# podmortem/operator

Hardware: AMD Instinct MI355X
Metric: pod-failure analyses/sec (whole node) + p50 explanation latency, 8B TP=1 (higher is better)
Workload: dtype bf16

## Files before the change

### csrc/bindings.cpp

```cpp
#include <torch/extension.h>
#include <c10/hip/HIPStream.h>
#include <ATen/hip/impl/HIPGuardImplMasqueradingAsCUDA.h>
#include <ATen/hip/impl/HIPStreamMasqueradingAsCUDA.h>

#include "kernels/kernels.h"
#include "kernels/scan.h"

namespace {

using oamd::bf16_t;

hipStream_t cur_stream() { return c10::hip::getCurrentHIPStreamMasqueradingAsCUDA().stream(); }

#define CHECK_DEV(t) TORCH_CHECK((t).is_cuda(), #t " must be a GPU tensor")
#define CHECK_CONTIG(t) TORCH_CHECK((t).is_contiguous(), #t " must be contiguous")
#define CHECK_DT(t, dt) TORCH_CHECK((t).scalar_type() == (dt), #t " has wrong dtype ", (t).scalar_type())
#define CHECK_BF16(t) CHECK_DT(t, at::kBFloat16)
#define ROWMAJOR_VEC(t) \
  TORCH_CHECK((t).dim() == 2 && (t).stride(1) == 1 && (t).stride(0) % 8 == 0, #t " must be [rows, cols] row-major with 16-B aligned rows")
#define RC(call)                                                           \
  do {                                                                     \
    int rc__ = (call);                                                     \
    TORCH_CHECK(rc__ == 0, "kernel launch failed: " #call " rc=", rc__);   \
  } while (0)
// ... 212 lines not shown

void gemm_tile(const at::Tensor& x, const at::Tensor& w, const c10::optional<at::Tensor>& y_opt,
               const c10::optional<at::Tensor>& bias, bool silu_gu, int64_t variant, int64_t splits,
               const c10::optional<at::Tensor>& partial) {
  CHECK_DEV(x); CHECK_BF16(x); CHECK_BF16(w); CHECK_CONTIG(x); CHECK_CONTIG(w);
  TORCH_CHECK(x.dim() == 2 && w.dim() == 2, "x [M,K], w [N,K]");
  const int64_t M = x.size(0), K = x.size(1), N = w.size(0);
  TORCH_CHECK(w.size(1) == K, "gemm_tile: w [N, K] must match x [M, K]");
  TORCH_CHECK(M >= 1 && K >= 64 && K % 64 == 0 && N % 16 == 0, "gemm_tile: K % 64 == 0, N % 16 == 0");
  TORCH_CHECK(splits >= 1 && splits <= 64 && K % (64 * splits) == 0, "gemm_tile: K % (64 * splits) == 0");
  bf16_t* yp = nullptr;
  int64_t ldy = silu_gu ? N / 2 : N;
  if (y_opt.has_value()) {
    const at::Tensor& y = *y_opt;
    CHECK_BF16(y);
    TORCH_CHECK(y.dim() == 2 && y.size(0) == M && y.size(1) == (silu_gu ? N / 2 : N) && y.stride(1) == 1 &&
                    y.stride(0) % 4 == 0,
                "gemm_tile: y [M, N] (N/2 with silu_gu), unit column stride, 8-B aligned rows");
    TORCH_CHECK(reinterpret_cast<uintptr_t>(y.data_ptr()) % 8 == 0, "gemm_tile: y must be 8-B aligned");
    TORCH_CHECK(splits == 1 || silu_gu || y.stride(0) == N, "gemm_tile: split-K reduce needs a contiguous y");
    yp = ptr<bf16_t>(y);
    ldy = y.stride(0);
  } else {
    TORCH_CHECK(splits > 1 && !silu_gu, "y may be omitted only for split-K slabs summed by the consumer");
  }
  TORCH_CHECK(!silu_gu || (N % 128 == 0 && !bias.has_value()), "gemm_tile: SwiGLU needs N % 128, no bias");
  TORCH_CHECK(splits == 1 || !bias.has_value(), "gemm_tile: no bias with split-K");
  if (bias.has_value()) {
    CHECK_BF16(*bias); CHECK_CONTIG(*bias);
    TORCH_CHECK(bias->numel() == N, "gemm_tile: bias [N]");
  }
  float* pp = nullptr;
  if (splits > 1) {
    TORCH_CHECK(partial.has_value(), "gemm_tile: split-K needs a partial buffer");
    CHECK_DT(*partial, at::kFloat); CHECK_CONTIG(*partial);
    TORCH_CHECK(partial->numel() >= splits * M * N, "gemm_tile: partial buffer too small");
    pp = partial->data_ptr<float>();
  }
  TORCH_CHECK(M * K < (1LL << 40) && N * K < (1LL << 40) && M < (1LL << 31) && N < (1LL << 31), "gemm too large");
  const c10::hip::HIPGuardMasqueradingAsCUDA g(x.device());
  RC(oamd::gemm_tile(ptr<bf16_t>(x), ptr<bf16_t>(w), yp, optr<bf16_t>(bias), (int)M, (int)N, (int)K, (int)ldy,
                     silu_gu, (int)variant, (int)splits, pp, cur_stream()));
}

void gemm_pp(const at::Tensor& x, const at::Tensor& w, const c10::optional<at::Tensor>& y_opt,
             const c10::optional<at::Tensor>& p, int64_t splits, int64_t bm, bool silu_gu, bool nt, bool one_seg,
             const c10::optional<at::Tensor>& sk_ws, const c10::optional<at::Tensor>& sk_flags) {
  CHECK_DEV(x); CHECK_BF16(x); CHECK_BF16(w); CHECK_CONTIG(x); CHECK_CONTIG(w);
  TORCH_CHECK(x.dim() == 2 && w.dim() == 2 && w.size(1) == x.size(1), "x [M,K], w [N,K]");
  const int64_t M = x.size(0), K = x.size(1), N = w.size(0);
  TORCH_CHECK(M >= 1 && N % 128 == 0, "gemm_pp: N % 128 == 0");
  TORCH_CHECK(bm == 128 || bm == 256, "gemm_pp: bm in {128, 256}");
  TORCH_CHECK(splits >= 1 && splits <= 32 && K % (64 * splits) == 0, "gemm_pp: K % (64 * splits) == 0");
  TORCH_CHECK(!silu_gu || splits == 1, "gemm_pp: fused SwiGLU needs splits == 1");
  bf16_t* yp = nullptr;
  if (y_opt.has_value()) {
    CHECK_BF16(*y_opt); CHECK_CONTIG(*y_opt);
    TORCH_CHECK(y_opt->dim() == 2 && y_opt->size(0) == M && y_opt->size(1) == (silu_gu ? N / 2 : N), "gemm_pp: y");
    yp = ptr<bf16_t>(*y_opt);
  } else {
    TORCH_CHECK(splits > 1 && !silu_gu, "y may be omitted only for split-K slabs summed by the consumer");
  }
  float* pp = nullptr;
  if (splits > 1) {
    TORCH_CHECK(p.has_value(), "split-K needs a partial buffer");
    CHECK_DT(*p, at::kFloat); CHECK_CONTIG(*p);
    TORCH_CHECK(p->numel() >= splits * M * N, "partial buffer too small");
    pp = p->data_ptr<float>();
  }
  TORCH_CHECK(M * K < (1LL << 40) && N * K < (1LL << 40), "gemm too large");
  const c10::hip::HIPGuardMasqueradingAsCUDA g(x.device());
  float* wsp = nullptr;
  int* flp = nullptr;
  if (sk_ws.has_value() || sk_flags.has_value()) {
    TORCH_CHECK(sk_ws.has_value() && sk_flags.has_value(), "gemm_pp: stream-K needs sk_ws and sk_flags");
    CHECK_DEV(*sk_ws); CHECK_DEV(*sk_flags); CHECK_CONTIG(*sk_ws); CHECK_CONTIG(*sk_flags);
    CHECK_DT(*sk_ws, at::kFloat); CHECK_DT(*sk_flags, at::kInt);
    TORCH_CHECK(sk_ws->numel() >= (N / 128) * 32768 && sk_flags->numel() >= N / 128, "gemm_pp: stream-K workspace too small");
    wsp = sk_ws->data_ptr<float>();
    flp = sk_flags->data_ptr<int>();
  }
  RC(oamd::gemm_pp(ptr<bf16_t>(x), ptr<bf16_t>(w), yp, pp, (int)M, (int)N, (int)K, (int)splits, (int)bm, silu_gu, nt,
                   cur_stream(), one_seg, wsp, flp));
}

void gemm_skinny(const at::Tensor& x, const at::Tensor& w, const c10::optional<at::Tensor>& y_opt,
                 const c10::optional<at::Tensor>& p, int64_t splits, bool silu_gu) {
  CHECK_DEV(x); CHECK_BF16(x); CHECK_BF16(w); CHECK_CONTIG(x); CHECK_CONTIG(w);
  TORCH_CHECK(x.dim() == 2 && w.dim() == 2 && w.size(1) == x.size(1), "x [M,K], w [N,K]");
  const int64_t M = x.size(0), K = x.size(1), N = w.size(0);
  TORCH_CHECK(M >= 1 && M <= 32, "gemm_skinny: M must be 1..32");
  TORCH_CHECK(N % (silu_gu ? 128 : 16) == 0, "gemm_skinny: N % 16 (128 for the fused SwiGLU)");
  TORCH_CHECK(splits >= 1 && splits <= 8 && K % (128 * splits) == 0, "gemm_skinny: K % (128 * splits)");
  TORCH_CHECK(!silu_gu || splits == 1, "fused SwiGLU needs splits = 1");
  bf16_t* yp = nullptr;
  if (y_opt.has_value()) {
    CHECK_BF16(*y_opt); CHECK_CONTIG(*y_opt);
    TORCH_CHECK(y_opt->dim() == 2 && y_opt->size(0) == M && y_opt->size(1) == (silu_gu ? N / 2 : N), "gemm shapes");
    yp = ptr<bf16_t>(*y_opt);
  } else {
    TORCH_CHECK(splits > 1 && !silu_gu, "y may be omitted only for split-K slabs summed by the consumer");
  }
  float* pp = nullptr;
  if (splits > 1) {
    TORCH_CHECK(p.has_value(), "split-K needs a partial buffer");
    CHECK_DT(*p, at::kFloat); CHECK_CONTIG(*p);
    TORCH_CHECK(p->numel() >= splits * M * N, "partial buffer too small");
    TORCH_CHECK((M * N) % 4 == 0 || yp == nullptr, "split-K reduce needs M * N % 4 == 0");
    pp = p->data_ptr<float>();
  }
  TORCH_CHECK(N * K < (1LL << 40) && M * K < (1LL << 31), "gemm too large");
  const c10::hip::HIPGuardMasqueradingAsCUDA g(x.device());
  RC(oamd::gemm_skinny(ptr<bf16_t>(x), ptr<bf16_t>(w), yp, pp, (int)M, (int)N, (int)K, (int)splits, silu_gu,
                       cur_stream()));
}

void quantize_fp8(const at::Tensor& x, at::Tensor& q, at::Tensor& sx) {
  CHECK_DEV(x); CHECK_BF16(x); CHECK_CONTIG(q); CHECK_CONTIG(sx); CHECK_DT(sx, at::kFloat);
  TORCH_CHECK(x.dim() == 2 && x.stride(1) == 1, "x must be [M, K] row-major");
  TORCH_CHECK(q.scalar_type() == at::kByte || q.scalar_type() == at::kFloat8_e4m3fn, "q must be uint8 / e4m3fn");
  const int64_t M = x.size(0), K = x.size(1);
  TORCH_CHECK(q.numel() == M * K && sx.numel() == M && K % 8 == 0, "quantize_fp8 shapes");
  const c10::hip::HIPGuardMasqueradingAsCUDA g(x.device());
  RC(oamd::quantize_fp8_rows(ptr<bf16_t>(x), static_cast<uint8_t*>(q.data_ptr()), ptr<float>(sx), (int)M, (int)K,
                             x.stride(0), cur_stream()));
}

void silu_quantize_fp8(const at::Tensor& gu, at::Tensor& q, at::Tensor& sx, const c10::optional<at::Tensor>& slabs,
                       int64_t splits) {
  CHECK_DEV(gu); CHECK_CONTIG(q); CHECK_CONTIG(sx); CHECK_DT(sx, at::kFloat);
  TORCH_CHECK(gu.dim() == 2 && gu.stride(1) == 1, "gu must be [M, 2I] row-major");
  TORCH_CHECK(q.scalar_type() == at::kByte || q.scalar_type() == at::kFloat8_e4m3fn, "q must be uint8 / e4m3fn");
  const int64_t M = gu.size(0), I = gu.size(1) / 2;
  TORCH_CHECK(gu.size(1) % 128 == 0 && I <= 16384, "silu_quantize_fp8: 2I % 128 == 0, I <= 16384");
  TORCH_CHECK(q.numel() == M * I && sx.numel() == M, "silu_quantize_fp8 shapes");
  const float* pp = nullptr;
  if (slabs.has_value()) {
    CHECK_DT(*slabs, at::kFloat); CHECK_CONTIG(*slabs);
    TORCH_CHECK(splits >= 1 && slabs->numel() >= splits * M * 2 * I, "slabs: fp32 [splits, M, 2I]");
    pp = slabs->data_ptr<float>();
  } else {
    CHECK_BF16(gu);
  }
  const c10::hip::HIPGuardMasqueradingAsCUDA g(gu.device());
  RC(oamd::silu_quantize_fp8(pp != nullptr ? nullptr : ptr<bf16_t>(gu), pp, (int)splits,
                             static_cast<uint8_t*>(q.data_ptr()), ptr<float>(sx), (int)M, (int)I,
                             pp != nullptr ? 2 * I : gu.stride(0), cur_stream()));
}

void gemm_fp8(const at::Tensor& x8, const at::Tensor& w8, const at::Tensor& sx, const at::Tensor& sw, at::Tensor& y,
              const c10::optional<at::Tensor>& p, int64_t splits, int64_t bn, int64_t bm, bool reduce) {
  CHECK_DEV(x8); CHECK_CONTIG(x8); CHECK_CONTIG(w8); CHECK_CONTIG(sx); CHECK_CONTIG(sw); CHECK_BF16(y);
  CHECK_CONTIG(y); CHECK_DT(sx, at::kFloat); CHECK_DT(sw, at::kFloat);
  for (auto* t : {&x8, &w8})
    TORCH_CHECK(t->scalar_type() == at::kByte || t->scalar_type() == at::kFloat8_e4m3fn, "fp8 operands");
  TORCH_CHECK(x8.dim() == 2 && w8.dim() == 2, "x8 [M,K], w8 [N,K]");
  const int64_t M = x8.size(0), K = x8.size(1), N = w8.size(0);
  TORCH_CHECK(w8.size(1) == K && y.size(0) == M && y.size(1) == N && sx.numel() == M && sw.numel() == N,
              "gemm_fp8 shapes");
  TORCH_CHECK((bn == 64 || bn == 128) && N % bn == 0, "gemm_fp8: N % bn");
  TORCH_CHECK(bm == 64 || bm == 128 || bm == 256, "gemm_fp8: bm in {64,128,256}");
  TORCH_CHECK(splits >= 1 && splits <= 16 && K % 128 == 0 && K / 128 >= splits, "gemm_fp8: K % 128, 1 <= splits <= min(16, K / 128)");
  float* pp = nullptr;
  if (splits > 1) {
    TORCH_CHECK(p.has_value() && p->scalar_type() == at::kFloat && p->numel() >= splits * M * N,
                "split-K needs an fp32 partial buffer");
// ... 150 lines not shown
                        ptr<int>(work_seq), ptr<int>(work_q0), (int)work_seq.numel(), (int)q.size(1),
                        (int)k.size(1), 128, (float)scale, (int)variant, cur_stream(), pkp, pvp, pfx));
}

void sample(const at::Tensor& logits, const at::Tensor& temperature, const at::Tensor& seeds,
            const at::Tensor& positions, at::Tensor& out, int64_t col_offset,
            const c10::optional<at::Tensor>& out_val) {
  CHECK_DEV(logits);
  TORCH_CHECK(logits.dim() == 2 && logits.stride(1) == 1, "logits must be [rows, vocab] row-major");
  TORCH_CHECK(logits.scalar_type() == at::kFloat || logits.scalar_type() == at::kBFloat16, "logits dtype");
  const int64_t rows = logits.size(0);
  CHECK_DT(temperature, at::kFloat); CHECK_DT(seeds, at::kLong); CHECK_DT(positions, at::kLong); CHECK_DT(out, at::kLong);
  TORCH_CHECK(temperature.numel() == rows && seeds.numel() == rows && positions.numel() == rows && out.numel() == rows,
              "sampler per-row tensor shape");
  if (out_val.has_value()) {
    CHECK_DT(*out_val, at::kFloat);
    TORCH_CHECK(out_val->numel() == rows, "out_val shape");
  }
  const c10::hip::HIPGuardMasqueradingAsCUDA g(logits.device());
  RC(oamd::sample_tokens(logits.data_ptr(), logits.scalar_type() == at::kBFloat16, logits.stride(0), (int)rows,
                         (int)logits.size(1), ptr<float>(temperature), ptr<int64_t>(seeds), ptr<int64_t>(positions),
                         ptr<int64_t>(out), col_offset, optr<float>(out_val), cur_stream()));
}

}

void graph_launch(int64_t exec, int64_t count, int64_t stream) {
  TORCH_CHECK(exec != 0 && count >= 0, "graph_launch: bad graph / count");
  hipError_t err = hipSuccess;
  {
    pybind11::gil_scoped_release nogil;
    for (int64_t i = 0; i < count && err == hipSuccess; ++i)
      err = hipGraphLaunch(reinterpret_cast<hipGraphExec_t>(exec), reinterpret_cast<hipStream_t>(stream));
  }
  TORCH_CHECK(err == hipSuccess, "hipGraphLaunch failed: ", hipGetErrorString(err));
}

void register_scan_bindings(pybind11::module_& m);
void register_comm_bindings(pybind11::module_& m);

PYBIND11_MODULE(_C, m) {
  m.doc() = "operator_amd gfx950 kernels";
  m.def("rmsnorm", &rmsnorm, "RMSNorm with optional fused residual add (and split-K slab sum)", pybind11::arg("x"),
        pybind11::arg("residual"), pybind11::arg("w"), pybind11::arg("y"), pybind11::arg("eps"),
        pybind11::arg("partial") = pybind11::none(), pybind11::arg("splits") = 1, pybind11::arg("tiled_out") = false);
  m.def("gemm_xr", &gemm_xr, pybind11::arg("xt"), pybind11::arg("w"), pybind11::arg("y") = pybind11::none(),
        pybind11::arg("p") = pybind11::none(), pybind11::arg("splits") = 1, pybind11::arg("epi") = 1);
  m.def("tile_rows", &tile_rows, pybind11::arg("x"), pybind11::arg("xt"));
  m.def("silu_mul", &silu_mul, pybind11::arg("gu"), pybind11::arg("out"), pybind11::arg("block") = 0);
  m.def("embedding", &embedding);
  m.def("rope_kv", &rope_kv, pybind11::arg("qkv"), pybind11::arg("pos"), pybind11::arg("cos"),
        pybind11::arg("sin"), pybind11::arg("Hq"), pybind11::arg("Hkv"), pybind11::arg("q_out"),
        pybind11::arg("k_out"), pybind11::arg("v_out"), pybind11::arg("k_cache"), pybind11::arg("v_cache"),
        pybind11::arg("slots"), pybind11::arg("partial") = pybind11::none(), pybind11::arg("splits") = 1,
        pybind11::arg("bias") = pybind11::none(), pybind11::arg("k_scale") = 1.0, pybind11::arg("v_scale") = 1.0);
  m.def("attn_decode", &attn_decode, pybind11::arg("q"), pybind11::arg("k_cache"), pybind11::arg("v_cache"),
        pybind11::arg("block_tables"), pybind11::arg("seq_lens"), pybind11::arg("out"), pybind11::arg("o_part"),
        pybind11::arg("ml_part"), pybind11::arg("num_splits"), pybind11::arg("scale"), pybind11::arg("variant") = 0,
        pybind11::arg("k_scale") = 1.0, pybind11::arg("v_scale") = 1.0, pybind11::arg("q8") = pybind11::none(),
        pybind11::arg("sx") = pybind11::none(), pybind11::arg("rope_x") = pybind11::none(),
        pybind11::arg("rope_splits") = 1, pybind11::arg("pos") = pybind11::none(), pybind11::arg("cos") = pybind11::none(),
        pybind11::arg("sin") = pybind11::none(), pybind11::arg("slots") = pybind11::none(),
        pybind11::arg("bias") = pybind11::none());
  m.def("decode_slots", &decode_slots);
  m.def("decode_advance", &decode_advance);
  m.def("quantize_fp8", &quantize_fp8);
  m.def("silu_quantize_fp8", &silu_quantize_fp8, pybind11::arg("gu"), pybind11::arg("q"), pybind11::arg("sx"),
        pybind11::arg("slabs") = pybind11::none(), pybind11::arg("splits") = 1);
  m.def("score_events", &score_events);
  m.def("gemm_fp8", &gemm_fp8, pybind11::arg("x8"), pybind11::arg("w8"), pybind11::arg("sx"), pybind11::arg("sw"),
        pybind11::arg("y"), pybind11::arg("p") = pybind11::none(), pybind11::arg("splits") = 1,
        pybind11::arg("bn") = 64, pybind11::arg("bm") = 64, pybind11::arg("reduce") = true);
  m.def("gemm_decode", &gemm_decode, pybind11::arg("x"), pybind11::arg("w"), pybind11::arg("y"),
        pybind11::arg("p") = pybind11::none(), pybind11::arg("splits") = 1, pybind11::arg("bn") = 64,
        pybind11::arg("bm") = 0, pybind11::arg("silu_gu") = false, pybind11::arg("w_tiled") = false,
        pybind11::arg("stages") = 3);
  m.def("gemm_tile", &gemm_tile, pybind11::arg("x"), pybind11::arg("w"), pybind11::arg("y"),
        pybind11::arg("bias") = pybind11::none(), pybind11::arg("silu_gu") = false, pybind11::arg("variant") = 0,
        pybind11::arg("splits") = 1, pybind11::arg("partial") = pybind11::none());
  m.def("gemm_pp", &gemm_pp, pybind11::arg("x"), pybind11::arg("w"), pybind11::arg("y"),
        pybind11::arg("p") = pybind11::none(), pybind11::arg("splits") = 1, pybind11::arg("bm") = 256,
        pybind11::arg("silu_gu") = false, pybind11::arg("nt") = true, pybind11::arg("one_seg") = false,
        pybind11::arg("sk_ws") = pybind11::none(), pybind11::arg("sk_flags") = pybind11::none());
  m.def("gemm_pp_sk_grid", &oamd::gemm_pp_sk_grid, pybind11::arg("tiles"), pybind11::arg("steps"));
  m.def("gemm_skinny", &gemm_skinny, pybind11::arg("x"), pybind11::arg("w"), pybind11::arg("y"),
        pybind11::arg("p") = pybind11::none(), pybind11::arg("splits") = 1, pybind11::arg("silu_gu") = false);
  m.def("attn_prefill", &attn_prefill, pybind11::arg("q"), pybind11::arg("k"), pybind11::arg("v"),
        pybind11::arg("o"), pybind11::arg("cu_seqlens"), pybind11::arg("work_seq"), pybind11::arg("work_q0"),
        pybind11::arg("scale"), pybind11::arg("block_q") = 64, pybind11::arg("pk") = pybind11::none(),
        pybind11::arg("pv") = pybind11::none(), pybind11::arg("seq_pfx") = pybind11::none());
  m.def("attn_prefill_block_q", &oamd::attn_prefill_block_q);
  m.def("sample", &sample, pybind11::arg("logits"), pybind11::arg("temperature"), pybind11::arg("seeds"),
        pybind11::arg("positions"), pybind11::arg("out"), pybind11::arg("col_offset") = 0,
        pybind11::arg("out_val") = pybind11::none());
  m.def("graph_launch", &graph_launch, pybind11::arg("graph_exec"), pybind11::arg("count"), pybind11::arg("stream"));
  register_scan_bindings(m);
  register_comm_bindings(m);
  m.attr("ARCH") = "gfx950";
}
```

### csrc/kernels/kernels.h

```cpp
#pragma once
#include <hip/hip_runtime.h>
#include <stdint.h>

namespace oamd {
typedef uint16_t bf16_t;

int rmsnorm(const bf16_t* x, bf16_t* residual, const bf16_t* w, bf16_t* y, int rows, int hidden,
            int64_t x_stride, int64_t r_stride, int64_t y_stride, float eps, const float* xp, int S,
            hipStream_t stream);
int silu_mul(const bf16_t* gu, bf16_t* out, int64_t rows, int inter, int block, int64_t in_stride,
             int64_t out_stride, hipStream_t stream);
int decode_slots(const int* bt, const int64_t* pos, const int* ctx, int64_t* slots, int64_t* spos, int B,
                 int max_pages, int page_size, hipStream_t stream);
int decode_advance(const int64_t* tok, int64_t* ids, int64_t* hist, int64_t* pos, int* ctx, int64_t* step, int B,
                   int ms, hipStream_t stream);
int embedding(const int64_t* ids, const bf16_t* table, bf16_t* out, int tokens, int hidden,
              int64_t vocab, hipStream_t stream);
int rope_kv(const bf16_t* qkv, int64_t qkv_stride, const int64_t* pos, const float* cos_t,
            const float* sin_t, int tokens, int Hq, int Hkv, int head_dim, bf16_t* q_out,
            bf16_t* k_out, bf16_t* v_out, void* k_cache, void* v_cache, const int64_t* slots,
            int page_size, int64_t max_pos, const float* xp, int S, const bf16_t* bias,
            bool fp8_cache, float k_scale, float v_scale, hipStream_t stream);
int gemm_decode(const bf16_t* X, const bf16_t* W, bf16_t* Y, float* P, int M, int N, int K, int S, int BN,
                int BM, bool silu_gu, bool w_tiled, int stages, hipStream_t stream);

int gemm_tile(const bf16_t* X, const bf16_t* W, bf16_t* Y, const bf16_t* bias, int M, int N, int K, int ldy,
              bool silu_gu, int variant, int S, float* P, hipStream_t stream);
int gemm_pp(const bf16_t* X, const bf16_t* W, bf16_t* Y, float* P, int M, int N, int K, int S, int bm, bool silu_gu,
            bool nt, hipStream_t stream, bool one_seg = false, float* ws = nullptr, int* flags = nullptr);
int gemm_pp_sk_grid(int tiles, int steps);
int gemm_xr(const bf16_t* Xt, const bf16_t* W, bf16_t* Y, float* P, int M, int N, int K, int S, int epi,
            hipStream_t stream);
int tile_rows(const bf16_t* x, bf16_t* xt, int rows, int K, hipStream_t stream);
int splitk_reduce(const float* P, bf16_t* Y, int64_t MN, int S, hipStream_t stream);
int gemm_skinny(const bf16_t* X, const bf16_t* W, bf16_t* Y, float* P, int M, int N, int K, int S, bool silu_gu,
                hipStream_t stream);

int gemm_fp8(const uint8_t* X, const uint8_t* W, const float* sx, const float* sw, bf16_t* Y, float* P, int M,
             int N, int K, int S, int BN, int BM, hipStream_t stream);
int quantize_fp8_rows(const bf16_t* x, uint8_t* q, float* sx, int M, int K, int64_t ld, hipStream_t stream);
int silu_quantize_fp8(const bf16_t* gu, const float* P, int S, uint8_t* q, float* sx, int M, int inter, int64_t ld,
                      hipStream_t stream);

int score_events(const int64_t* keys, const int* hit_doc, const int* doc_ptr, int n_hits, int n_docs,
                 const int* prim_ptr, const int* prim_pat, const int* ev_ptr, const int* ev_doc_ptr,
                 const int* sec_ptr, const int* sec_matcher, const double* sec_w, const int* sec_win,
                 const double* conf, const int* severity, int num_matchers, double significance, double* ev_score,
                 int* ev_pat, int* ev_line, int* order, int* summary, hipStream_t stream);

struct DecRope {
  const float* xp;
  const bf16_t* row;
  int64_t row_stride;
  int S;
  int64_t slab;
  const bf16_t* bias;
  const int64_t* pos;
  const float* cos_t;
  const float* sin_t;
  int64_t max_pos;
  const int64_t* slots;
  float k_inv, v_inv;
};

int attn_decode(const bf16_t* q, const void* k_cache, const void* v_cache, bool fp8, float k_scale, float v_scale,
                const int* block_tables, const int* seq_lens, bf16_t* out, float* o_part, float* ml_part, int B,
                int Hq, int Hkv, int head_dim, int page_size, int max_pages, int num_splits, float scale, int variant,
                hipStream_t stream, uint8_t* q8 = nullptr, float* sx = nullptr, const DecRope* rope = nullptr);
int attn_prefill_block_q(int Hq, int Hkv, int variant);
int attn_prefill(const bf16_t* q, const bf16_t* k, const bf16_t* v, bf16_t* o, const int* cu_seqlens,
                 const int* work_seq, const int* work_q0, int num_work, int Hq, int Hkv, int head_dim,
                 float scale, int variant, hipStream_t stream,
                 const bf16_t* pk = nullptr, const bf16_t* pv = nullptr, const int* seq_pfx = nullptr);
int sample_tokens(const void* logits, bool logits_bf16, int64_t stride, int rows, int vocab,
                  const float* temperature, const int64_t* seeds, const int64_t* positions,
                  int64_t* out_tokens, int64_t col_offset, float* out_val, hipStream_t stream);

size_t car_buffer_bytes(size_t cap_bytes, int world);
int car_alloc(size_t cap_bytes, int world, void** base, void* handle_out );
int car_open(const void* handle, void** ptr);
int car_close(void* ptr);
int car_free(void* base);
int car_host_flag(uint32_t** host, uint32_t** dev);
void car_free_host_flag(uint32_t* host);
int car_error(const uint32_t* host);
int car_reset(void* base, size_t bytes, uint32_t* host);
constexpr int kCarOneShot = 0, kCarTwoShot = 1, kCarOneShotFence = 2, kCarLL = 3;
int car_all_reduce_rmsnorm(const void* in, const float* slabs, int S, bf16_t* residual, const bf16_t* w, bf16_t* y,
                           uint8_t* q8, float* sx, int rows, int hidden, float eps, int rank, int world,
                           void* const* bases, size_t cap_bytes, int blocks, uint32_t* herr_dev, double timeout_s,
                           int proto, hipStream_t stream);
int car_all_reduce(const void* in, void* out, int64_t bytes, bool bf16, int rank, int world, void* const* bases,
                   size_t cap_bytes, int blocks, uint32_t* herr_dev, double timeout_s, int proto,
                   hipStream_t stream);

}
```

### operator_amd/ops/__init__.py

```python
from __future__ import annotations

import json
import os

import torch
import torch.nn.functional as F

from . import reference
from ._native import kernels, native_available, patterns

__all__ = [
    "rmsnorm", "silu_mul", "embedding", "rope_kv", "attn_prefill", "attn_decode", "attn_decode_rope", "sample",
    "kernels", "patterns", "native_available", "reference", "prefill_work_list", "prefill_block_q", "prefill_variant", "decode_splits",
    "decode_workspace", "linear", "gemm_splits", "gemm_plan", "gate_up_silu", "interleave_gate_up",
    "quantize_fp8", "silu_quantize_fp8", "linear_fp8", "fp8_plan", "SplitK", "linear_tile", "tile_ok", "BLAS_CALLS",
]

DECODE_MIN_SPLIT_TOKENS = int(os.environ.get("OAMD_DECODE_MIN_SPLIT", "256"))
DECODE_TARGET_BLOCKS = int(os.environ.get("OAMD_DECODE_TARGET_BLOCKS", "256"))
DECODE_ATTN_VARIANT = int(os.environ.get("OAMD_DECODE_ATTN_VARIANT", "0"))


class SplitK:

    __slots__ = ("p", "S", "shape", "device", "dtype", "is_cuda")

    def __init__(self, p: torch.Tensor, S: int, M: int, N: int):
        self.p, self.S, self.shape = p, S, (M, N)
        self.device, self.dtype, self.is_cuda = p.device, torch.bfloat16, True

    def materialize(self) -> torch.Tensor:
        M, N = self.shape
        return self.p[: self.S * M * N].view(self.S, M, N).sum(0).to(torch.bfloat16)


def rmsnorm(x, w: torch.Tensor, eps: float, residual: torch.Tensor | None = None,
            out: torch.Tensor | None = None) -> torch.Tensor:
    if isinstance(x, SplitK):
        M, N = x.shape
        y = out if out is not None else torch.empty(M, N, dtype=torch.bfloat16, device=x.device)
        kernels().rmsnorm(y, residual, w, y, eps, x.p, x.S)
        return y
    if not x.is_cuda:
        y, r = reference.rmsnorm(x, w, eps, residual)
        if residual is not None:
            residual.copy_(r)
        if out is not None:
            out.copy_(y)
            return out
        return y
    y = out if out is not None else torch.empty_like(x)
    kernels().rmsnorm(x, residual, w, y, eps)
    return y


def silu_mul(gu: torch.Tensor, out: torch.Tensor | None = None, block: int | None = None) -> torch.Tensor:
    if not gu.is_cuda:
        r = reference.silu_mul(gu, block)
        if out is not None:
            out.copy_(r)
            return out
        return r
    inter = gu.shape[1] // 2
    o = out if out is not None else torch.empty(gu.shape[0], inter, dtype=gu.dtype, device=gu.device)
    kernels().silu_mul(gu, o, block or 0)
    return o


GU_BLOCK = 64


def interleave_gate_up(g: torch.Tensor, u: torch.Tensor, block: int = GU_BLOCK) -> torch.Tensor:
    inter, H = g.shape
    return torch.stack([g.reshape(inter // block, block, H), u.reshape(inter // block, block, H)], 1).reshape(
        2 * inter, H).contiguous()


def gate_up_silu(x: torch.Tensor, wgu: torch.Tensor, block: int | None) -> torch.Tensor:
    M, K = x.shape
    N = wgu.shape[0]
    if (x.is_cuda and block == 64 and x.dtype == torch.bfloat16 and M <= SKINNY_MAX_M and N % 128 == 0
            and K % 128 == 0 and x.is_contiguous() and wgu.is_contiguous()
            and skinny_plan(M, N, K) is not None and _gemm_table_get().get(("silu", M, N, K)) != "blas"):
        y = torch.empty(M, N // 2, dtype=x.dtype, device=x.device)
        kernels().gemm_skinny(x, wgu, y, None, 1, True)
        return y
    if (x.is_cuda and block == 64 and x.dtype == torch.bfloat16 and M % 64 == 0 and M <= 256 and N % 128 == 0
            and K % 64 == 0 and x.is_contiguous() and wgu.is_contiguous()):
        t = _gemm_table_get().get(("silu", M, N, K))
        if isinstance(t, str) and t.startswith("pp"):
            y = torch.empty(M, N // 2, dtype=x.dtype, device=x.device)
            bm = int(t[2:])
            ws, fl = _pp_sk_workspace(x.device, N // 128) if (bm == 256 and PP_STREAM_K) else (None, None)
            kernels().gemm_pp(x, wgu, y, None, 1, bm, True, True, False, ws, fl)
            return y
        if t != "blas":
            bm = t[0] if t else row_tile(M)
            ns = t[1] if t and len(t) > 1 else 3
            y = torch.empty(M, N // 2, dtype=x.dtype, device=x.device)
            kernels().gemm_decode(x, wgu, y, None, 1, 128, bm, True, False, ns)
            return y
    if block == 64 and tile_ok(x, wgu) and N % 128 == 0:
        return linear_tile(x, wgu, silu_gu=True)
    return silu_mul(linear(x, wgu), block=block)


PP_STREAM_K = os.environ.get("OAMD_PP_STREAM_K", "0") == "1"
_PP_SK_WS: dict = {}


def _pp_sk_workspace(device, tiles: int):
    key = (str(device), tiles)
    ws = _PP_SK_WS.get(key)
    if ws is None:
        ws = (torch.empty(tiles * 32768, dtype=torch.float32, device=device),
              torch.zeros(tiles, dtype=torch.int32, device=device))
        _PP_SK_WS[key] = ws
    return ws


def embedding(ids: torch.Tensor, table: torch.Tensor, out: torch.Tensor | None = None) -> torch.Tensor:
    if not ids.is_cuda:
        r = reference.embedding(ids, table)
        if out is not None:
            out.copy_(r)
            return out
        return r
    o = out if out is not None else torch.empty(ids.numel(), table.shape[1], dtype=table.dtype, device=ids.device)
    kernels().embedding(ids, table, o)
    return o


def rope_kv(qkv: torch.Tensor, pos: torch.Tensor, cos: torch.Tensor, sin: torch.Tensor, Hq: int, Hkv: int,
            k_cache: torch.Tensor | None = None, v_cache: torch.Tensor | None = None,
            slots: torch.Tensor | None = None, want_kv: bool = True,
            q_out: torch.Tensor | None = None, bias: torch.Tensor | None = None,
            k_scale: float = 1.0, v_scale: float = 1.0):
    if isinstance(qkv, SplitK):
        T = qkv.shape[0]
        D = cos.shape[1] * 2
        dev = qkv.device
        q = q_out if q_out is not None else torch.empty(T, Hq, D, dtype=torch.bfloat16, device=dev)
        k = torch.empty(T, Hkv, D, dtype=torch.bfloat16, device=dev) if want_kv else None
        v = torch.empty(T, Hkv, D, dtype=torch.bfloat16, device=dev) if want_kv else None
        kernels().rope_kv(q, pos, cos, sin, Hq, Hkv, q, k, v, k_cache, v_cache, slots, qkv.p, qkv.S, bias,
                          k_scale, v_scale)
        return q, k, v
    if not qkv.is_cuda:
        if bias is not None:
            qkv = (qkv.float() + bias.float()).to(qkv.dtype)
        q, k, v = reference.rope_kv(qkv, pos, cos, sin, Hq, Hkv, k_cache, v_cache, slots, k_scale, v_scale)
        if q_out is not None:
            q_out.copy_(q.reshape(q_out.shape))
            q = q_out
        return q, (k if want_kv else None), (v if want_kv else None)
    T = qkv.shape[0]
    D = cos.shape[1] * 2
    q = q_out if q_out is not None else torch.empty(T, Hq, D, dtype=qkv.dtype, device=qkv.device)
    k = torch.empty(T, Hkv, D, dtype=qkv.dtype, device=qkv.device) if want_kv else None
    v = torch.empty(T, Hkv, D, dtype=qkv.dtype, device=qkv.device) if want_kv else None
    kernels().rope_kv(qkv, pos, cos, sin, Hq, Hkv, q, k, v, k_cache, v_cache, slots, None, 1, bias, k_scale, v_scale)
    return q, k, v


_PREFILL_VARIANTS = {"v1": 1, "v2": 2, "v3": 3, "v4": 4}


def prefill_variant(Hq: int, Hkv: int) -> int:
    G = Hq // Hkv if Hkv and Hq % Hkv == 0 else 0
    want = _PREFILL_VARIANTS.get(os.environ.get("OAMD_PREFILL_ATTN", ""), 4 if 1 <= G <= 4 else 3)
    if want == 2 and G not in (1, 2, 4, 8):
        want = 3
    if want == 4 and G > 4:
        want = 3
    return want if 1 <= G <= 8 else 1


def prefill_block_q(Hq: int, Hkv: int, variant: int | None = None) -> int:
    v = prefill_variant(Hq, Hkv) if variant is None else variant
    if v == 1:
        return 64
    G = Hq // Hkv
    return (16 if v == 2 else 32) * ((4 if v == 4 else 8) // G)


def prefill_work_list(seq_lens: list[int], block_q: int = 64) -> tuple[list[int], list[int]]:
    items = []
    for s, L in enumerate(seq_lens):
        for q0 in range(0, L, block_q):
            items.append((q0, s))
# ... 96 lines not shown
    if t == "blas":
        return None
    if t is not None:
        return int(t)
    S = 1
    while (N // 16) * S < 512 and S < 8 and K % (128 * S * 2) == 0:
        S *= 2
    return S


PREFILL_BLAS = os.environ.get("OAMD_PREFILL_BLAS", "0") == "1"
BLAS_CALLS = {"n": 0}
BLAS_PLANNED = {"n": 0}


def _blas(x: torch.Tensor, w: torch.Tensor, out: torch.Tensor | None, bias: torch.Tensor | None,
          planned: bool = False):
    if x.is_cuda and planned:
        BLAS_PLANNED["n"] += 1
    elif x.is_cuda:
        BLAS_CALLS["n"] += 1
        if os.environ.get("OAMD_FORBID_BLAS") == "1":
            raise RuntimeError(f"hipBLASLt fallback for x {tuple(x.shape)} {x.dtype}, w {tuple(w.shape)} "
                               "(OAMD_FORBID_BLAS=1)")
    if out is not None:
        return F.linear(x, w, bias, out=out) if bias is None else out.copy_(F.linear(x, w, bias))
    return F.linear(x, w, bias)


def tile_ok(x: torch.Tensor, w: torch.Tensor) -> bool:
    return (x.is_cuda and x.dtype == torch.bfloat16 and w.dtype == torch.bfloat16 and x.dim() == 2
            and x.is_contiguous() and w.is_contiguous() and x.shape[1] % 64 == 0 and w.shape[0] % 16 == 0
            and x.shape[0] >= 1)


def tile_out_ok(out: torch.Tensor | None) -> bool:
    return out is None or (out.dim() == 2 and out.stride(1) == 1 and out.stride(0) % 4 == 0
                           and out.data_ptr() % 8 == 0 and out.dtype == torch.bfloat16)


def linear_tile(x: torch.Tensor, w: torch.Tensor, out: torch.Tensor | None = None,
                bias: torch.Tensor | None = None, silu_gu: bool = False) -> torch.Tensor:
    M = x.shape[0]
    N = w.shape[0]
    y = out if out is not None else torch.empty(M, N // 2 if silu_gu else N, dtype=x.dtype, device=x.device)
    kernels().gemm_tile(x, w, y, bias, silu_gu)
    return y


def linear(x: torch.Tensor, w: torch.Tensor, out: torch.Tensor | None = None, splits: int | None = None,
           partial: torch.Tensor | None = None, bn: int | None = None, bm: int | None = None,
           defer_reduce: bool = False, stages: int | None = None, bias: torch.Tensor | None = None):
    M, K = x.shape
    N = w.shape[0]
    plan = None
    if bias is not None:
        if tile_ok(x, w) and tile_out_ok(out):
            return linear_tile(x, w, out, bias)
        return _blas(x, w, out, bias)
    if x.is_cuda and bm is None and bn is None and splits is None and _measured_blas(M, N, K):
        return _blas(x, w, out, None)
    if PREFILL_BLAS and x.is_cuda and M > 256 and N < LM_HEAD_MIN_N and splits is None and x.dtype == torch.bfloat16:
        return _blas(x, w, out, None, planned=True)
    if (x.is_cuda and x.dtype == torch.bfloat16 and x.is_contiguous() and w.is_contiguous() and M <= SKINNY_MAX_M
            and bm is None and bn is None):
        S = splits or skinny_plan(M, N, K)
        if S is not None:
            if S > 1 and (partial is None or partial.numel() < S * M * N):
                partial = torch.empty(S * M * N, dtype=torch.float32, device=x.device)
            if defer_reduce and S > 1 and out is None:
                kernels().gemm_skinny(x, w, None, partial, S, False)
                return SplitK(partial, S, M, N)
            y = out if out is not None else torch.empty(M, N, dtype=x.dtype, device=x.device)
            kernels().gemm_skinny(x, w, y, partial if S > 1 else None, S, False)
            return y
    if x.is_cuda and x.dtype == torch.bfloat16 and x.is_contiguous() and w.is_contiguous():
        plan = gemm_plan(M, N, K)
        if plan is None and (splits or bn or bm) and M % 64 == 0 and M <= 256 and N % 64 == 0 and K % 64 == 0:
            plan = (row_tile(M), 64, 1)
    if plan is None:
        if tile_ok(x, w) and tile_out_ok(out):
            return linear_tile(x, w, out)
        return _blas(x, w, out, None)
    bm, bn, S = bm or plan[0], bn or plan[1], splits or plan[2]
    ns = stages or (plan[3] if len(plan) > 3 else 3)
    if S > 1 and (partial is None or partial.numel() < S * M * N):
        partial = torch.empty(S * M * N, dtype=torch.float32, device=x.device)
    if defer_reduce and S > 1 and out is None:
        kernels().gemm_decode(x, w, None, partial, S, bn, bm, False, False, ns)
        return SplitK(partial, S, M, N)
    y = out if out is not None else torch.empty(M, N, dtype=x.dtype, device=x.device)
    kernels().gemm_decode(x, w, y, partial if S > 1 else None, S, bn, bm, False, False, ns)
    return y


FP8_MAX = 448.0


def quantize_fp8(x: torch.Tensor) -> tuple[torch.Tensor, torch.Tensor]:
    M, K = x.shape
    if x.is_cuda and x.dtype == torch.bfloat16 and K % 8 == 0:
        q = torch.empty(M, K, dtype=torch.float8_e4m3fn, device=x.device)
        sx = torch.empty(M, dtype=torch.float32, device=x.device)
        kernels().quantize_fp8(x.contiguous(), q, sx)
        return q, sx
    xf = x.float()
    amax = xf.abs().amax(1)
    sx = torch.where(amax > 0, amax / FP8_MAX, torch.ones_like(amax))
    return (xf / sx[:, None]).to(torch.float8_e4m3fn), sx


def silu_quantize_fp8(gu, block: int | None = GU_BLOCK) -> tuple[torch.Tensor, torch.Tensor]:
    M, N2 = gu.shape
    inter = N2 // 2
    if gu.is_cuda and block == GU_BLOCK and inter <= 16384 and N2 % 128 == 0:
        q = torch.empty(M, inter, dtype=torch.float8_e4m3fn, device=gu.device)
        sx = torch.empty(M, dtype=torch.float32, device=gu.device)
        if isinstance(gu, SplitK):
            kernels().silu_quantize_fp8(torch.empty(M, N2, dtype=torch.bfloat16, device=gu.device), q, sx,
                                        gu.p, gu.S)
            return q, sx
        if gu.stride(1) == 1:
            kernels().silu_quantize_fp8(gu, q, sx)
            return q, sx
    if isinstance(gu, SplitK):
        gu = gu.materialize()
    return quantize_fp8(silu_mul(gu, block=block))


def _fp8_overrides() -> dict:
    out = {}
    for item in filter(None, os.environ.get("OAMD_FP8_PLANS", "").split(";")):
        shape, plan = item.split("=")
        n, k = (int(v) for v in shape.split("x"))
        out[(n, k)] = tuple(int(v) for v in plan.split(","))
    return out


_FP8_OVERRIDES = _fp8_overrides()


def fp8_plan(M: int, N: int, K: int) -> tuple[int, int, int]:
    if (N, K) in _FP8_OVERRIDES:
        return _FP8_OVERRIDES[(N, K)]
    bm = 64 if M <= 64 else 128 if M <= 128 else 256
    bn = 128 if N % 128 == 0 and N // 128 >= 192 else 64
    mt = -(-M // bm)
    S = 1
    for s in (1, 2, 4, 8):
        if K % (128 * s):
            break
        S = s
        if (N // bn) * s * mt >= 256:
            break
    return bm, bn, S


def linear_fp8(x: torch.Tensor | tuple[torch.Tensor, torch.Tensor], w8: torch.Tensor, sw: torch.Tensor,
               out: torch.Tensor | None = None, plan: tuple[int, int, int] | None = None,
               defer_reduce: bool = False):
    q, sx = x if isinstance(x, tuple) else quantize_fp8(x)
    M, K = q.shape
    N = w8.shape[0]
    if not q.is_cuda:
        y = (q.float() * sx[:, None]) @ (w8.float() * sw[:, None]).t()
        return out.copy_(y) if out is not None else y.to(torch.bfloat16 if isinstance(x, tuple) else x.dtype)
    bm, bn, S = plan or fp8_plan(M, N, K)
    y = out if out is not None else torch.empty(M, N, dtype=torch.bfloat16, device=q.device)
    part = torch.empty(S * M * N, dtype=torch.float32, device=q.device) if S > 1 else None
    if defer_reduce and S > 1 and out is None:
# ... 88 lines not shown
```

Baseline: 31.23.

## Add hand-scheduled triple-buffered 256x128 bf16 GEMM kernel for M=256 decode

Adds a new gemm_w4 kernel for 256-row bf16 GEMMs. Each block covers a 256x128 output tile with four waves. It triple-buffers direct global-to-LDS buffer loads and hand-interleaves MFMA instructions with LDS reads and DMA issues using sched barriers, and supports a fused SwiGLU epilogue and split-K partials. The Python dispatch routes to it when the gemm table marks a shape 'w4', on by default via OAMD_DEC_GEMM_W4. The aim is to better overlap memory traffic with matrix math than the existing pp/decode kernels, at the cost of a rigid shape restriction and fragile inline-asm scheduling.

```diff
diff --git a/csrc/bindings.cpp b/csrc/bindings.cpp
--- a/csrc/bindings.cpp
+++ b/csrc/bindings.cpp
@@ -318,6 +318,36 @@
   }
   RC(oamd::gemm_pp(ptr<bf16_t>(x), ptr<bf16_t>(w), yp, pp, (int)M, (int)N, (int)K, (int)splits, (int)bm, silu_gu, nt,
                    cur_stream(), one_seg, wsp, flp));
+}
+
+void gemm_w4(const at::Tensor& x, const at::Tensor& w, const c10::optional<at::Tensor>& y_opt,
+             const c10::optional<at::Tensor>& p, int64_t splits, bool silu_gu) {
+  CHECK_DEV(x); CHECK_BF16(x); CHECK_BF16(w); CHECK_CONTIG(x); CHECK_CONTIG(w);
+  TORCH_CHECK(x.dim() == 2 && w.dim() == 2 && w.size(1) == x.size(1), "x [M,K], w [N,K]");
+  const int64_t M = x.size(0), K = x.size(1), N = w.size(0);
+  TORCH_CHECK(M == 256, "gemm_w4: M == 256");
+  TORCH_CHECK(N >= 128 && N % 128 == 0, "gemm_w4: N % 128 == 0");
+  TORCH_CHECK(K >= 64 && K % 64 == 0 && K < (1LL << 22), "gemm_w4: K % 64 == 0, K < 2^22");
+  TORCH_CHECK(splits >= 1 && splits <= 16 && splits <= K / 64, "gemm_w4: 1 <= splits <= min(16, K / 64)");
+  TORCH_CHECK(!silu_gu || splits == 1, "gemm_w4: fused SwiGLU needs splits == 1");
+  bf16_t* yp = nullptr;
+  if (y_opt.has_value()) {
+    CHECK_DEV(*y_opt); CHECK_BF16(*y_opt); CHECK_CONTIG(*y_opt);
+    TORCH_CHECK(y_opt->dim() == 2 && y_opt->size(0) == M && y_opt->size(1) == (silu_gu ? N / 2 : N), "gemm_w4: y");
+    yp = ptr<bf16_t>(*y_opt);
+  } else {
+    TORCH_CHECK(splits > 1 && !silu_gu, "y may be omitted only for split-K slabs summed by the consumer");
+  }
+  float* pp = nullptr;
+  if (splits > 1) {
+    TORCH_CHECK(p.has_value(), "split-K needs a partial buffer");
+    CHECK_DEV(*p); CHECK_DT(*p, at::kFloat); CHECK_CONTIG(*p);
+    TORCH_CHECK(p->numel() >= splits * M * N, "partial buffer too small");
+    pp = p->data_ptr<float>();
+  }
+  TORCH_CHECK(N * K < (1LL << 40), "gemm too large");
+  const c10::hip::HIPGuardMasqueradingAsCUDA g(x.device());
+  RC(oamd::gemm_w4(ptr<bf16_t>(x), ptr<bf16_t>(w), yp, pp, (int)M, (int)N, (int)K, (int)splits, silu_gu, cur_stream()));
 }
 
 void gemm_skinny(const at::Tensor& x, const at::Tensor& w, const c10::optional<at::Tensor>& y_opt,
@@ -634,6 +664,8 @@
         pybind11::arg("p") = pybind11::none(), pybind11::arg("splits") = 1, pybind11::arg("bm") = 256,
         pybind11::arg("silu_gu") = false, pybind11::arg("nt") = true, pybind11::arg("one_seg") = false,
         pybind11::arg("sk_ws") = pybind11::none(), pybind11::arg("sk_flags") = pybind11::none());
+  m.def("gemm_w4", &gemm_w4, pybind11::arg("x"), pybind11::arg("w"), pybind11::arg("y"),
+        pybind11::arg("p") = pybind11::none(), pybind11::arg("splits") = 1, pybind11::arg("silu_gu") = false);
   m.def("gemm_pp_sk_grid", &oamd::gemm_pp_sk_grid, pybind11::arg("tiles"), pybind11::arg("steps"));
   m.def("gemm_skinny", &gemm_skinny, pybind11::arg("x"), pybind11::arg("w"), pybind11::arg("y"),
         pybind11::arg("p") = pybind11::none(), pybind11::arg("splits") = 1, pybind11::arg("silu_gu") = false);
diff --git a/csrc/kernels/gemm_w4.hip b/csrc/kernels/gemm_w4.hip
--- /dev/null
+++ b/csrc/kernels/gemm_w4.hip
@@ -0,0 +1,231 @@
+#include <type_traits>
+
+#include "common.h"
+#include "kernels.h"
+
+namespace oamd {
+
+namespace {
+
+constexpr int kM = 256;
+constexpr int kBK = 64;
+constexpr int kXBytes = 32768;
+constexpr int kBuf = 49152;
+constexpr int kPre = 9;
+
+enum { kStore = 0, kPartial = 1, kSilu = 2 };
+enum { kSteady = 0, kPenult = 1, kLast = 2 };
+
+template <int N>
+__device__ __forceinline__ void vmw() {
+  asm volatile("s_waitcnt vmcnt(%0)" ::"n"(N) : "memory");
+}
+
+__device__ __forceinline__ void seg() {
+  __builtin_amdgcn_sched_barrier(0);
+  __builtin_amdgcn_s_barrier();
+  __builtin_amdgcn_sched_barrier(0);
+}
+
+__device__ __forceinline__ void mfma_tied(f32x4& acc, const u16x8& a, const u16x8& b) {
+  asm volatile("v_mfma_f32_16x16x32_bf16 %0, %1, %2, %0" : "+a"(acc) : "v"(a), "v"(b));
+}
+
+__device__ __forceinline__ uint2 pack4(f32x4 v) { return make_uint2(pack_bf2(v[0], v[1]), pack_bf2(v[2], v[3])); }
+
+}
+
+template <int EPI>
+__global__ void __launch_bounds__(256) gemm_w4_kernel(const bf16_t* __restrict__ X, const bf16_t* __restrict__ W,
+                                                      bf16_t* __restrict__ Y, float* __restrict__ P, int N, int K,
+                                                      int S) {
+  __shared__ __attribute__((aligned(1024))) char lds[3 * kBuf];
+  const int tid = threadIdx.x, lane = tid & 63;
+  const int w = __builtin_amdgcn_readfirstlane(tid >> 6);
+  const int wm = w >> 1, wn = w & 1;
+  const int kz = blockIdx.x % S, n0 = (blockIdx.x / S) * 128;
+  const int TK = K / kBK;
+  const int t0 = kz * TK / S;
+  const int T = (kz + 1) * TK / S - t0;
+
+  const int lrow = lane >> 3, lslot = lane & 7;
+  uint32_t vo[8];
+#pragma unroll
+  for (int q = 0; q < 8; ++q) {
+    const int row = 8 * (w + 4 * q) + lrow;
+    vo[q] = ((uint32_t)row * (uint32_t)K + (uint32_t)((lslot ^ ((row >> 1) & 7)) * 8)) * 2u;
+  }
+  const bf16_t* wbase = W + (int64_t)n0 * K;
+  const int xbytes = kM * K * 2, wbytes = 128 * K * 2;
+  auto dma_x = [&](const bf16_t* b, int nb, int off, int kt, int q) {
+    char* dst = lds + off + (w + 4 * q) * 1024;
+    __builtin_amdgcn_raw_ptr_buffer_load_lds(__builtin_amdgcn_make_buffer_rsrc((void*)b, (short)0, nb, 0x00020000),
+                                             (__attribute__((address_space(3))) void*)dst, 16, (int)vo[q],
+                                             (t0 + kt) * (kBK * 2), 0, 0);
+  };
+  auto dma_w = [&](const bf16_t* b, int nb, int off, int kt, int q) {
+    char* dst = lds + off + kXBytes + (w + 4 * q) * 1024;
+    __builtin_amdgcn_raw_ptr_buffer_load_lds(__builtin_amdgcn_make_buffer_rsrc((void*)b, (short)0, nb, 0x00020000),
+                                             (__attribute__((address_space(3))) void*)dst, 16, (int)vo[q],
+                                             (t0 + kt) * (kBK * 2), 0, 2);
+  };
+  auto piece = [&](int off, int kt, int p) {
+    if (p < 4) dma_w(wbase, wbytes, off, kt, p);
+    else dma_x(X, xbytes, off, kt, p - 4);
+  };
+
+  const int l15 = lane & 15, lq = lane >> 4, sw = (l15 >> 1) & 7;
+  const int xo0 = (wm * 128 + l15) * 128 + ((lq ^ sw) << 4);
+  const int xo1 = (wm * 128 + l15) * 128 + (((4 + lq) ^ sw) << 4);
+  const int wo0 = kXBytes + (wn * 32 + l15) * 128 + ((lq ^ sw) << 4);
+  const int wo1 = kXBytes + (wn * 32 + l15) * 128 + (((4 + lq) ^ sw) << 4);
+  auto rd = [&](int off, int h, u16x8 (&xf)[8], u16x8 (&wf)[4], int r) {
+    const int wrow = (r >> 1) * 64 + (r & 1) * 16;
+    if (r < 4) wf[r] = *reinterpret_cast<const u16x8*>(lds + off + (h ? wo1 : wo0) + wrow * 128);
+    else xf[r - 4] = *reinterpret_cast<const u16x8*>(lds + off + (h ? xo1 : xo0) + (r - 4) * 2048);
+  };
+
+  f32x4 acc[8][4];
+#pragma unroll
+  for (int i = 0; i < 8; ++i)
+#pragma unroll
+    for (int j = 0; j < 4; ++j) acc[i][j] = f32x4{0.f, 0.f, 0.f, 0.f};
+#pragma unroll
+  for (int i = 0; i < 8; ++i)
+#pragma unroll
+    for (int j = 0; j < 4; ++j) asm volatile("" : "+a"(acc[i][j]));
+  asm volatile("s_nop 4");
+  u16x8 xa[8], wa[4], xb[8], wb[4];
+
+  auto mm_b = [&](int m) {
+    const int i = m < 8 ? m : (m < 11 ? 0 : 1 + (m - 11) / 3);
+    const int j = m < 8 ? 0 : (m < 11 ? m - 7 : 1 + (m - 11) % 3);
+    mfma_tied(acc[i][j], wb[j], xb[i]);
+  };
+  auto head = [&](auto mode_c, int cur, int tgt, int kt2) {
+    constexpr int MODE = decltype(mode_c)::value;
+#pragma unroll
+    for (int m = 0; m < 32; ++m) {
+      mfma_tied(acc[m >> 2][m & 3], wa[m & 3], xa[m >> 2]);
+      __builtin_amdgcn_sched_barrier(0);
+      if (m < 24 && m % 2 == 0) rd(cur, 1, xb, wb, m >> 1);
+      if (MODE == kSteady && m % 5 == 3) piece(tgt, kt2, m / 5);
+      __builtin_amdgcn_sched_barrier(0);
+    }
+#pragma unroll
+    for (int m = 0; m < 12; ++m) {
+      mm_b(m);
+      __builtin_amdgcn_sched_barrier(0);
+      if (MODE == kSteady && m % 5 == 1) piece(tgt, kt2, 6 + m / 5);
+      __builtin_amdgcn_sched_barrier(0);
+    }
+    if constexpr (MODE != kLast) {
+      if constexpr (MODE == kSteady) vmw<kPre>(); else vmw<0>();
+      seg();
+    }
+  };
+  auto tail = [&](auto mode_c, int nxt, int tgt, int kt2) {
+    constexpr int MODE = decltype(mode_c)::value;
+#pragma unroll
+    for (int m = 12; m < 32; ++m) {
+      mm_b(m);
+      __builtin_amdgcn_sched_barrier(0);
+      if (MODE != kLast && m < 24) {
+        const int k = m - 12;
+        rd(nxt, 0, xa, wa, k == 0 ? 0 : (k == 1 ? 4 : (k < 5 ? k - 1 : k)));
+      }
+      if (MODE == kSteady && m >= 25 && (m - 25) % 3 == 0) piece(tgt, kt2, 9 + (m - 25) / 3);
+      __builtin_amdgcn_sched_barrier(0);
+    }
+  };
+
+#pragma unroll
+  for (int p = 0; p < 12; ++p) piece(0, 0, p);
+  if (T > 1) {
+#pragma unroll
+    for (int p = 0; p < 12; ++p) piece(kBuf, 1, p);
+    vmw<12>();
+  } else {
+    vmw<0>();
+  }
+  seg();
+#pragma unroll
+  for (int k = 0; k < 12; ++k) rd(0, 0, xa, wa, k == 0 ? 0 : (k == 1 ? 4 : (k < 5 ? k - 1 : k)));
+
+  int cur = 0, nxt = kBuf, tgt = 2 * kBuf;
+  auto rotate = [&]() {
+    const int c = cur;
+    cur = nxt;
+    nxt = tgt;
+    tgt = c;
+  };
+  constexpr std::integral_constant<int, kSteady> steady{};
+  constexpr std::integral_constant<int, kPenult> penult{};
+  constexpr std::integral_constant<int, kLast> last{};
+  if (T > 2) {
+    head(steady, cur, tgt, 2);
+    for (int t = 0; t + 3 < T; ++t) {
+      tail(steady, nxt, tgt, t + 2);
+      rotate();
+      head(steady, cur, tgt, t + 3);
+    }
+    tail(steady, nxt, tgt, T - 1);
+    rotate();
+  }
+  if (T > 1) {
+    head(penult, cur, tgt, 0);
+    tail(penult, nxt, tgt, 0);
+    rotate();
+  }
+  head(last, cur, tgt, 0);
+  tail(last, nxt, tgt, 0);
+
+  asm volatile("s_nop 7\n s_nop 7\n s_nop 7" ::: "memory");
+#pragma unroll
+  for (int i = 0; i < 8; ++i) {
+    const int tok = wm * 128 + i * 16 + l15;
+    if constexpr (EPI == kSilu) {
+#pragma unroll
+      for (int jj = 0; jj < 2; ++jj) {
+        const f32x4 gt = acc[i][jj], up = acc[i][2 + jj];
+        f32x4 o;
+#pragma unroll
+        for (int r = 0; r < 4; ++r) {
+          const float gg = bf2f(f2bf(gt[r]));
+          const float uu = bf2f(f2bf(up[r]));
+          o[r] = bf2f(f2bf(gg / (1.f + __expf(-gg)))) * uu;
+        }
+        const int col = (n0 >> 1) + wn * 32 + jj * 16 + 4 * lq;
+        *reinterpret_cast<uint2*>(Y + (int64_t)tok * (N >> 1) + col) = pack4(o);
+      }
+    } else {
+#pragma unroll
+      for (int j = 0; j < 4; ++j) {
+        const int col = n0 + (j >> 1) * 64 + wn * 32 + (j & 1) * 16 + 4 * lq;
+        if constexpr (EPI == kPartial)
+          *reinterpret_cast<f32x4*>(P + ((int64_t)kz * kM + tok) * N + col) = acc[i][j];
+        else
+          *reinterpret_cast<uint2*>(Y + (int64_t)tok * N + col) = pack4(acc[i][j]);
+      }
+    }
+  }
+}
+
+int gemm_w4(const bf16_t* X, const bf16_t* W, bf16_t* Y, float* P, int M, int N, int K, int S, bool silu_gu,
+            hipStream_t stream) {
+  if (M != kM || N < 128 || N % 128 != 0 || K < kBK || K % kBK != 0) return -1;
+  if ((int64_t)kM * K * 2 >= (1LL << 31)) return -2;
+  if (S < 1 || S > 16 || K / kBK < S) return -3;
+  if (S > 1 && P == nullptr) return -4;
+  if (silu_gu && S != 1) return -5;
+  if (S == 1 && Y == nullptr) return -6;
+  const int grid = (N / 128) * S;
+  if (silu_gu) gemm_w4_kernel<kSilu><<<grid, 256, 0, stream>>>(X, W, Y, P, N, K, S);
+  else if (S > 1) gemm_w4_kernel<kPartial><<<grid, 256, 0, stream>>>(X, W, Y, P, N, K, S);
+  else gemm_w4_kernel<kStore><<<grid, 256, 0, stream>>>(X, W, Y, P, N, K, S);
+  OAMD_LAUNCH_CHECK();
+  if (S > 1 && Y != nullptr) return splitk_reduce(P, Y, (int64_t)M * N, S, stream);
+  return 0;
+}
+
+}
diff --git a/csrc/kernels/kernels.h b/csrc/kernels/kernels.h
--- a/csrc/kernels/kernels.h
+++ b/csrc/kernels/kernels.h
@@ -29,6 +29,8 @@
 int gemm_pp(const bf16_t* X, const bf16_t* W, bf16_t* Y, float* P, int M, int N, int K, int S, int bm, bool silu_gu,
             bool nt, hipStream_t stream, bool one_seg = false, float* ws = nullptr, int* flags = nullptr);
 int gemm_pp_sk_grid(int tiles, int steps);
+int gemm_w4(const bf16_t* X, const bf16_t* W, bf16_t* Y, float* P, int M, int N, int K, int S, bool silu_gu,
+            hipStream_t stream);
 int gemm_xr(const bf16_t* Xt, const bf16_t* W, bf16_t* Y, float* P, int M, int N, int K, int S, int epi,
             hipStream_t stream);
 int tile_rows(const bf16_t* x, bf16_t* xt, int rows, int K, hipStream_t stream);
diff --git a/operator_amd/ops/__init__.py b/operator_amd/ops/__init__.py
--- a/operator_amd/ops/__init__.py
+++ b/operator_amd/ops/__init__.py
@@ -88,6 +88,14 @@
     if (x.is_cuda and block == 64 and x.dtype == torch.bfloat16 and M % 64 == 0 and M <= 256 and N % 128 == 0
             and K % 64 == 0 and x.is_contiguous() and wgu.is_contiguous()):
         t = _gemm_table_get().get(("silu", M, N, K))
+        if t == "w4":
+            if M != 256:
+                raise ValueError(f"gemm table: plan 'w4' on silu,{M},{N},{K}: gemm_w4 takes the 256-row bucket only")
+            if DEC_GEMM_W4:
+                y = torch.empty(M, N // 2, dtype=x.dtype, device=x.device)
+                kernels().gemm_w4(x, wgu, y, None, 1, True)
+                return y
+            t = "pp256"
         if isinstance(t, str) and t.startswith("pp"):
             y = torch.empty(M, N // 2, dtype=x.dtype, device=x.device)
             bm = int(t[2:])
@@ -106,6 +114,7 @@
 
 
 PP_STREAM_K = os.environ.get("OAMD_PP_STREAM_K", "0") == "1"
+DEC_GEMM_W4 = os.environ.get("OAMD_DEC_GEMM_W4", "1") != "0"
 _PP_SK_WS: dict = {}
 
 
@@ -368,10 +377,21 @@
         if tile_ok(x, w) and tile_out_ok(out):
             return linear_tile(x, w, out)
         return _blas(x, w, out, None)
+    if len(plan) > 4 and plan[4] == "w4" and (M != 256 or tuple(plan[:2]) != (256, 128)):
+        raise ValueError(f"gemm table: plan {plan} on {M},{N},{K}: gemm_w4 runs M = 256 as 256 x 128 tiles only")
+    w4 = (DEC_GEMM_W4 and len(plan) > 4 and plan[4] == "w4" and bm is None and bn is None
+          and splits is None and stages is None)
     bm, bn, S = bm or plan[0], bn or plan[1], splits or plan[2]
     ns = stages or (plan[3] if len(plan) > 3 else 3)
     if S > 1 and (partial is None or partial.numel() < S * M * N):
         partial = torch.empty(S * M * N, dtype=torch.float32, device=x.device)
+    if w4:
+        if defer_reduce and S > 1 and out is None:
+            kernels().gemm_w4(x, w, None, partial, S, False)
+            return SplitK(partial, S, M, N)
+        y = out if out is not None else torch.empty(M, N, dtype=x.dtype, device=x.device)
+        kernels().gemm_w4(x, w, y, partial if S > 1 else None, S, False)
+        return y
     if defer_reduce and S > 1 and out is None:
         kernels().gemm_decode(x, w, None, partial, S, bn, bm, False, False, ns)
         return SplitK(partial, S, M, N)
```

Result: faster. 31.65 (median of 6 runs) (+1.4%).
